# uzh-rpg/dagr

Hardware: NVIDIA H100
Metric: Mevents/sec (higher is better)
Workload: dtype f32

## Files before the change

dagr_b200/_lib.py:

```python
from __future__ import annotations

import ctypes as C
import os
from pathlib import Path

import torch

_PKG = Path(__file__).resolve().parent
_LIB_PATH = Path(os.environ["DAGR_B200_LIB"]) if os.environ.get("DAGR_B200_LIB") else _PKG / "libdagr_b200.so"
_lib = None

ELL = 16
KU = 15
TABW = 16
L1_TC_WFRAG_FLOATS = 8192

p = C.c_void_p
i32 = C.c_int32
i64 = C.c_int64
f32 = C.c_float


class Geom(C.Structure):
    _fields_ = [("W", i32), ("H", i32), ("B", i32), ("T", i32),
                ("r", i32), ("ncell", i32),
                ("dt_us", i32), ("K", i32), ("Q", i32),
                ("nx1", i32), ("ny1", i32),
                ("CW", i32), ("CH", i32), ("CP", i32),
                ("NK", i32),
                ("xkey", p), ("ykey", p), ("spiral", p), ("posx0", p), ("posy0", p), ("vx0", p), ("vy0", p), ("tabx", p), ("taby", p)]


class Grid(C.Structure):
    _fields_ = [("nx", i32), ("ny", i32), ("B", i32), ("W", i32), ("H", i32),
                ("posxr", p), ("posyr", p)]


class EventWs(C.Structure):
    _fields_ = [(k, i64) for k in ("key", "tmp", "count", "blocksums", "start", "perm", "ti", "xyb", "feat_s", "nbr", "off", "cellmask",
                                   "xa", "wl_hdr", "wl_ids", "x1")]


class PoolWs(C.Structure):
    _fields_ = [(k, i64) for k in ("acc", "possum", "ptmax", "pcnt", "pmask")]


class L1AParams(C.Structure):
    _fields_ = [("w", f32 * (KU * 3 * 16)), ("root", f32 * (3 * 16)),
# ... 15 lines not shown
    "dagr_abi_version": (C.c_int, []),
    "dagr_last_error": (C.c_char_p, []),
    "dagr_scan_blocks": (i64, [i64]),
    "dagr_check_config": (C.c_int, [C.POINTER(Geom), i64, C.c_int, C.c_int, C.c_char_p]),
    "dagr_event_workspace_bytes": (C.c_int, [C.POINTER(Geom), i64, C.POINTER(EventWs)]),
    "dagr_pool_workspace_bytes": (C.c_int, [i64, C.c_int, C.POINTER(PoolWs)]),
    "dagr_downsample_events": (C.c_int, [p, p, p, i64, C.c_int, C.c_int, C.c_int, C.c_int, p, p, p, p, p, p, p, p, p]),
    "dagr_compact_events": (C.c_int, [p, i64, p, p, p, p, C.c_int, C.c_int, p, p, p, p, p, p, p, p, p]),
    "dagr_ingest_events": (C.c_int, [p, p, p, p, i64, C.c_int, C.c_int, C.c_int, C.c_int, i64, C.c_int, p, p, p, p, p, p, p, p, p]),
    "dagr_denormalize_pos": (C.c_int, [p, i64, C.c_int, C.c_int, C.c_int, p, p]),
    "dagr_prepare_events": (C.c_int, [p, p, p, C.c_int, i64, C.c_int, C.c_int, C.c_int, p, p, p, p]),
    "dagr_graph_sort": (C.c_int, [C.POINTER(Geom), p, p, p, i64, p, p, p, p, p, p, p, p, p, p, p]),
    "dagr_graph_sort_ring": (C.c_int, [C.POINTER(Geom), p, p, p, i64, p, p, p, p, p, p, p, p, p, p, p, p]),
    "dagr_stream_push": (C.c_int, [p, p, p, p, p, i64, C.c_int, C.c_int, p]),
    "dagr_stream_push_multi": (C.c_int, [p, p, p, p, p, i64, C.c_int, C.c_int, p]),
    "dagr_graph_sort_rings": (C.c_int, [C.POINTER(Geom), p, p, p, i64, C.c_int, p, p, p, p, p, p, p, p, p, p, p, p]),
    "dagr_graph_search": (C.c_int, [C.POINTER(Geom), i64, p, p, p, p, p, p, p]),
    "dagr_l1_build": (C.c_int, [C.POINTER(Geom), i64, p, p, p, p, p, C.POINTER(L1AParams), p, C.c_int, p, p, p, p, p, p, C.c_int, p]),
    "dagr_xa_permute": (C.c_int, [i64, p, C.c_int, p, p, C.c_int, p]),
    "dagr_l1_x0_image": (C.c_int, [C.POINTER(Geom), i64, p, p, p, C.c_int, C.c_int, p, p]),
    "dagr_l1_x0_image_live": (C.c_int, [C.POINTER(Geom), i64, p, p, p, p, C.c_int, C.c_int, p, p]),
    "dagr_l1_conv_a_image": (C.c_int, [C.POINTER(Geom), i64, p, p, p, p, p, p, C.POINTER(L1ImgParams), p, p, p, p, C.c_int, p]),
    "dagr_voxel_sample_max": (C.c_int, [C.POINTER(Geom), i64, p, p, p, C.c_int, C.c_int, C.c_int, p, C.c_int, C.c_int, C.c_int, p]),
    "dagr_graph_export": (C.c_int, [C.POINTER(Geom), i64, p, p, p, p, p, p, p, p, i64, p]),
    "dagr_l1_conv_a": (C.c_int, [C.POINTER(Geom), i64, p, p, p, p, p, C.POINTER(L1AParams), p, p]),
    "dagr_l1_conv_b_pool": (C.c_int, [C.POINTER(Geom), i64, p, p, p, p, p, p, C.POINTER(L1BParams), p, p, p]),
    "dagr_l1_conv_b_pool_voxel": (C.c_int, [C.POINTER(Geom), i64, p, p, p, p, p, p, p, p, C.POINTER(L1BParams), p, C.c_int, p, p, p, p, p, p, p, C.c_int, p, p, C.c_int, p]),
    "dagr_l1_tc_weights": (C.c_int, [p, p, C.c_int, p]),
    "dagr_l1_conv_b_pool_voxel_tc": (C.c_int, [C.POINTER(Geom), i64, p, p, p, p, p, p, p, C.POINTER(L1BParams), p, p, C.c_int, p, p, p, p, p, p, p, C.c_int, p, p, C.c_int, p]),
    "dagr_l1_conv_a_image_tc": (C.c_int, [C.POINTER(Geom), i64, p, p, p, p, p, p, C.POINTER(L1ImgParams), p, p, p, p, p, C.c_int, p]),
    "dagr_pool1_finalize": (C.c_int, [C.POINTER(Geom), i64, p, p, p, p, C.c_int, p, p, p, p, p, p]),
    "dagr_grid_cat_pos": (C.c_int, [C.POINTER(Grid), p, p, p, C.c_int, p, p]),
    "dagr_grid_conv": (C.c_int, [C.POINTER(Grid), p, p, p, p, C.c_int, C.c_int, C.c_int, p, p, p, p, p, p, C.c_int, f32, f32, p, p]),
    "dagr_grid_linear_bn": (C.c_int, [i64, p, p, C.c_int, C.c_int, p, p, p, p, p]),
    "dagr_grid_pool": (C.c_int, [C.POINTER(Grid), C.POINTER(Grid), p, p, p, p, p, p, p, p, C.c_int, C.c_int,
                                 p, p, p, p, p, p, p, p]),
    "dagr_grid_pool_finalize": (C.c_int, [C.POINTER(Grid), C.c_int, C.c_int, p, p, p, p, p, p, p, p, p, p]),
    "dagr_grid_temporal_filter": (C.c_int, [C.POINTER(Grid), p, p, p, p]),
    "dagr_grid_to_dense": (C.c_int, [C.POINTER(Grid), p, p, C.c_int, C.c_int, p, p, p]),
    "dagr_head_decode": (C.c_int, [p, p, p, C.c_int, C.c_int, C.c_int, C.c_int, C.c_int, C.c_int, C.c_int, p, p]),
    "dagr_head_finish": (C.c_int, [C.POINTER(Grid), p, p, C.c_int, p, C.c_int, p, p, p, C.c_int, C.c_int, C.c_int, C.c_int, p, p]),
    "dagr_postprocess_nms": (C.c_int, [p, C.c_int, C.c_int, C.c_int, f32, f32, C.c_int, C.c_int, C.c_int, p, p, p]),
    "dagr_sample_features": (C.c_int, [p, C.c_int, C.c_int, C.c_int, C.c_int, p, p, p, i64, C.c_int, C.c_int, p,
                                       C.c_int, C.c_int, p]),
    "dagr_masked_lin": (C.c_int, [p, i64, p, p, p, p, C.c_int, C.c_int, C.c_int, p]),
    "dagr_masked_inplace_bn": (C.c_int, [p, i64, p, p, p, p, p, p, C.c_int, f32, p]),
    "dagr_masked_isdiff": (C.c_int, [p, i64, p, p, C.c_int, f32, f32, p]),
}

EXPORTS = tuple(_SIGS.keys())


def lib_path() -> Path:
    return _LIB_PATH


def load():
    global _lib
    if _lib is not None:
        return _lib
    if not os.environ.get("DAGR_B200_LIB"):
        from . import build as _build
        if _build.needs_build():
            try:
                _build.build(force=True)
            except Exception as e:
# ... 40 lines not shown
```

dagr_b200/csrc/coarse.cu:

```cuda
#include "common.cuh"

__device__ __forceinline__ float div_floor_f32(float a, float b)
{
    const float mod = fmodf(a, b);
    float div = __fdiv_rn(__fsub_rn(a, mod), b);
    if ((mod != 0.f) && ((b < 0.f) != (mod < 0.f))) div -= 1.f;
    float fl;
    if (div != 0.f) {
        fl = floorf(div);
        if (div - fl > 0.5f) fl += 1.f;
    } else {
        fl = copysignf(0.f, __fdiv_rn(a, b));
    }
    return fl;
}

__device__ __forceinline__ int round_to_pixel(float mean, int size)
{
    const float inv = __frcp_rn((float)size);
    const float q = div_floor_f32(__fadd_rn(mean, 1e-5f), inv);
    const int k = (int)q;
    return min(max(k, 0), size - 1);
}

// ... 284 lines not shown
            const int cell = cell0 + j;
            if (cell >= cells) continue;
            float v = 0.f;
            if (cnt[cell] > 0) {
#pragma unroll
                for (int w2 = 0; w2 < SK_WARPS; w2++) v += part[((size_t)w2 * CPB + j) * Cout + o];
                if (bias) v += bias[o];
                if (scale) v = fmaf(v, scale[o], shift[o]);
                if (skip) v += skip[(int64_t)cell * Cout + o];
                if (relu) v = fmaxf(v, 0.f);
            }
            out[(int64_t)cell * Cout + o] = v;
        }
    }
}

template <int CPB>
static int launch_grid_conv_sk(const dagr_grid_t *gr, const int32_t *cnt, const int32_t *pxy, const uint32_t *mask,
                               const float *xin, int ldin, int Cin, int Cout, const float *weight, const float *rootT, const float *bias,
                               const float *scale, const float *shift, const float *skip, int relu, float den_x, float den_y,
                               float *out, cudaStream_t st)
{
    const int cells = gr->B * gr->ny * gr->nx;
    const size_t a_bytes = (size_t)SK_SLOTS * Cin * CPB * sizeof(float), p_bytes = (size_t)SK_WARPS * CPB * Cout * sizeof(float);
    const size_t smem = (Cout <= 64) ? (a_bytes > p_bytes ? a_bytes : p_bytes) : a_bytes + p_bytes;
    if (smem > 200 * 1024) return -1;
    cudaError_t e = dagr_allow_smem(k_grid_conv_sk<CPB>, smem);
    if (e != cudaSuccess) return -2;
    k_grid_conv_sk<CPB><<<dagr_div_up(cells, CPB), SK_WARPS * 32, smem, st>>>(*gr, cnt, pxy, mask, xin, ldin, Cin, Cout, weight, rootT, bias,
                                                                            scale, shift, skip, relu, den_x, den_y, out);
    return 0;
}

extern "C" int dagr_grid_conv(const dagr_grid_t *gr, const int32_t *cnt, const int32_t *pxy, const uint32_t *mask,
                              const float *xin, int ldin, int Cin, int Cout, const float *weight, const float *rootT,
                              const float *bias, const float *scale, const float *shift, const float *skip, int relu,
                              float den_x, float den_y, float *out, void *stream)
{
    DAGR_CHECK_ARG(gr && Cin > 0 && Cout > 0 && (ldin == 0 || ldin >= Cin), "bad channels");
    if (ldin == 0) ldin = Cin;
    const int cells = gr->B * gr->ny * gr->nx;
    cudaStream_t st = (cudaStream_t)stream;
    static int n_sm = 0;
    if (n_sm == 0) {
        int dev = 0;
        DAGR_CUDA(cudaGetDevice(&dev));
        DAGR_CUDA(cudaDeviceGetAttribute(&n_sm, cudaDevAttrMultiProcessorCount, dev));
    }
    int rc = -1;
    const size_t per_cell = ((size_t)SK_SLOTS * Cin + (Cout <= 64 ? 0 : (size_t)SK_WARPS * Cout)) * sizeof(float);
    if (cells >= n_sm * 16 * 2 && per_cell * 16 <= 110 * 1024)
        rc = launch_grid_conv_sk<16>(gr, cnt, pxy, mask, xin, ldin, Cin, Cout, weight, rootT, bias, scale, shift, skip, relu, den_x, den_y, out, st);
    if (rc != 0 && cells >= n_sm * 4 && per_cell * 4 <= 160 * 1024)
        rc = launch_grid_conv_sk<4>(gr, cnt, pxy, mask, xin, ldin, Cin, Cout, weight, rootT, bias, scale, shift, skip, relu, den_x, den_y, out, st);
    if (rc != 0)
        rc = launch_grid_conv_sk<1>(gr, cnt, pxy, mask, xin, ldin, Cin, Cout, weight, rootT, bias, scale, shift, skip, relu, den_x, den_y, out, st);
    if (rc != 0) {
        const size_t smem = (size_t)GC_WARPS * GC_SLOTS * Cin * sizeof(float);
        DAGR_CHECK_ARG(smem <= 200 * 1024, "Cin too large for the grid conv kernels");
        DAGR_CUDA(dagr_allow_smem(k_grid_conv, smem));
        k_grid_conv<<<dagr_div_up(cells, GC_WARPS), GC_WARPS * 32, smem, st>>>(
            *gr, cnt, pxy, mask, xin, ldin, Cin, Cout, weight, rootT, bias, scale, shift, skip, relu, den_x, den_y, out);
    }
    DAGR_CHECK_LAUNCH();
    return DAGR_OK;
}

#define LB_CELLS 8
__global__ void __launch_bounds__(256)
k_grid_linear_bn(int64_t cells, const int32_t *__restrict__ cnt, const float *__restrict__ xin, int Cin,
                 int Cout, const float *__restrict__ wT, const float *__restrict__ scale,
                 const float *__restrict__ shift, float *__restrict__ out)
{
    extern __shared__ float s_x[];
    __shared__ int s_valid[LB_CELLS];
    const int64_t cell0 = (int64_t)blockIdx.x * LB_CELLS;
    for (int i = threadIdx.x; i < LB_CELLS * Cin; i += blockDim.x) {
        const int64_t cell = cell0 + i / Cin;
        s_x[i] = (cell < cells) ? xin[cell * Cin + i % Cin] : 0.f;
    }
    if (threadIdx.x < LB_CELLS) s_valid[threadIdx.x] = (cell0 + threadIdx.x < cells) && cnt[cell0 + threadIdx.x] > 0;
    __syncthreads();
    const int groups = LB_CELLS / 4;
    for (int t = threadIdx.x; t < Cout * groups; t += blockDim.x) {
        const int o = t % Cout, jg = t / Cout;
        const float *x0 = s_x + (size_t)(4 * jg) * Cin;
        float acc[4] = {0.f, 0.f, 0.f, 0.f};
        for (int c0 = 0; c0 < Cin; c0 += 8) {
            float w[8];
#pragma unroll
            for (int u = 0; u < 8; u++) w[u] = (c0 + u < Cin) ? __ldg(wT + (int64_t)(c0 + u) * Cout + o) : 0.f;
#pragma unroll
            for (int u = 0; u < 8; u++) {
                const int c = min(c0 + u, Cin - 1);
#pragma unroll
                for (int k = 0; k < 4; k++) acc[k] = fmaf(x0[(size_t)k * Cin + c], w[u], acc[k]);
            }
// ... 403 lines not shown
```

dagr_b200/csrc/common.cuh:

```cuda
#pragma once
#include <cuda_runtime.h>
#include <stdint.h>
#include <stdio.h>
#include "../../include/dagr_b200.h"

#ifndef __CUDA_ARCH__
#define DAGR_HOST 1
#endif

void dagr_set_error(const char *fmt, ...);

#define DAGR_CHECK_ARG(cond, msg)                                              \
    do { if (!(cond)) { dagr_set_error("%s: %s", __func__, msg); return DAGR_E_ARG; } } while (0)

#define DAGR_CHECK_LAUNCH()                                                    \
    do { cudaError_t e__ = cudaGetLastError();                                 \
         if (e__ != cudaSuccess) { dagr_set_error("%s: %s", __func__, cudaGetErrorString(e__)); \
                                   return DAGR_E_CUDA; } } while (0)

#define DAGR_CUDA(call)                                                        \
    do { cudaError_t e__ = (call);                                             \
         if (e__ != cudaSuccess) { dagr_set_error("%s: %s", __func__, cudaGetErrorString(e__)); \
                                   return DAGR_E_CUDA; } } while (0)

cudaError_t dagr_allow_smem_impl(const void *kernel, size_t bytes, bool max_carveout);
template <class K> static inline cudaError_t dagr_allow_smem(K kernel, size_t bytes, bool max_carveout = false)
{
    return dagr_allow_smem_impl(reinterpret_cast<const void *>(kernel), bytes, max_carveout);
}

static inline int dagr_div_up(int64_t a, int64_t b) { return (int)((a + b - 1) / b); }

int scan_exclusive(const int *in, int *out, int64_t n, int *blocksums, cudaStream_t st);

#define XA_SWZ(p) ((int)(((p) >> 2) & 1))

__device__ __forceinline__ uint32_t enc_ordered(float f)
{
    uint32_t u = __float_as_uint(f);
    return (u & 0x80000000u) ? ~u : (u | 0x80000000u);
}
__device__ __forceinline__ float dec_ordered(uint32_t e)
{
    uint32_t u = (e & 0x80000000u) ? (e & 0x7fffffffu) : ~e;
    return __uint_as_float(u);
}

__device__ __forceinline__ float2 ffma2(float2 a, float2 b, float2 c) { return make_float2(fmaf(a.x, b.x, c.x), fmaf(a.y, b.y, c.y)); }

__device__ __forceinline__ void spline_basis2(float ax, float ay, int ks, float w[4], int slot[4])
{
    float vx = ax * (float)(ks - 1), vy = ay * (float)(ks - 1);
    float fx = vx - floorf(vx), fy = vy - floorf(vy);
    int ix = (int)vx, iy = (int)vy;
#pragma unroll
    for (int s = 0; s < 4; s++) {
        int kx = s & 1, ky = (s >> 1) & 1;
        int sx = (ix + kx) % ks, sy = (iy + ky) % ks;
        if (sx < 0) sx += ks;
        if (sy < 0) sy += ks;
        slot[s] = sx + ks * sy;
        w[s] = (kx ? fx : 1.f - fx) * (ky ? fy : 1.f - fy);
    }
}
```

dagr_b200/csrc/conv_l1.cu:

```cuda
#include <string.h>
#include "common.cuh"

#define L1_THREADS 128

struct L1Smem {
    float *tab;
    float *posx;
    float *posy;
    short *sp;
};

__device__ __forceinline__ L1Smem l1_smem_init(const dagr_geom_t &g, const float *__restrict__ tab, unsigned char *raw)
{
    L1Smem s;
    s.tab = (float *)raw;
    s.posx = s.tab + g.ncell * DAGR_TABW;
    s.posy = s.posx + g.W;
    s.sp = (short *)(s.posy + g.H);
    for (int i = threadIdx.x; i < g.ncell * DAGR_TABW; i += blockDim.x) s.tab[i] = tab[i];
    for (int i = threadIdx.x; i < g.W; i += blockDim.x) s.posx[i] = g.posx0[i];
    for (int i = threadIdx.x; i < g.H; i += blockDim.x) s.posy[i] = g.posy0[i];
    for (int i = threadIdx.x; i < g.ncell; i += blockDim.x)
        s.sp[i] = (short)(((int)g.spiral[2 * i] & 0xff) | ((int)g.spiral[2 * i + 1] << 8));
    __syncthreads();
// ... 258 lines not shown
    asm volatile("fence.mbarrier_init.release.cluster;" ::: "memory");
}
__device__ __forceinline__ void mbar_expect_tx(uint64_t *bar, uint32_t bytes)
{
    asm volatile("mbarrier.arrive.expect_tx.shared::cta.b64 _, [%0], %1;" ::"r"(smem_u32(bar)), "r"(bytes) : "memory");
}
__device__ __forceinline__ void mbar_wait(uint64_t *bar, uint32_t parity)
{
    asm volatile(
        "{\n"
        ".reg .pred p;\n"
        "WAIT_%=:\n"
        "mbarrier.try_wait.parity.shared::cta.b64 p, [%0], %1;\n"
        "@p bra DONE_%=;\n"
        "bra WAIT_%=;\n"
        "DONE_%=:\n"
        "}\n" ::"r"(smem_u32(bar)), "r"(parity) : "memory");
}
__device__ __forceinline__ void tma_bulk_g2s(void *dst_smem, const void *src_gmem, uint32_t bytes, uint64_t *bar)
{
    asm volatile("cp.async.bulk.shared::cluster.global.mbarrier::complete_tx::bytes [%0], [%1], %2, [%3];" ::"r"(smem_u32(dst_smem)),
                 "l"(src_gmem), "r"(bytes), "r"(smem_u32(bar))
                 : "memory");
}

struct CB2Tile {
    int run_start[3], run_len[3], run_off[3];
};

#ifndef CB2_TC
#define CB2_TC 1
#endif
#define CB2_TC_KSTEPS 16

__device__ __forceinline__ uint32_t tf32_rna(float x)
{
    uint32_t r;
    asm("cvt.rna.tf32.f32 %0, %1;" : "=r"(r) : "f"(x));
    return r;
}
__device__ __forceinline__ void mma_tf32(float2 &c01, float2 &c23, const uint32_t a[4], uint32_t b0, uint32_t b1)
{
    asm("mma.sync.aligned.m16n8k8.row.col.f32.tf32.tf32.f32 {%0, %1, %2, %3}, {%4, %5, %6, %7}, {%8, %9}, {%0, %1, %2, %3};"
        : "+f"(c01.x), "+f"(c01.y), "+f"(c23.x), "+f"(c23.y)
        : "r"(a[0]), "r"(a[1]), "r"(a[2]), "r"(a[3]), "r"(b0), "r"(b1));
}

__device__ __forceinline__ void cb2_tc_kstep(float *xt, const float a[8], const float4 *__restrict__ wf, float2 o2[8])
{
    const int lane = threadIdx.x & 31;
    const float4 w0 = __ldg(wf), w1 = __ldg(wf + 1);
    const uint32_t bh[2][2] = {{__float_as_uint(w0.x), __float_as_uint(w0.y)}, {__float_as_uint(w1.x), __float_as_uint(w1.y)}};
    const uint32_t bl[2][2] = {{__float_as_uint(w0.z), __float_as_uint(w0.w)}, {__float_as_uint(w1.z), __float_as_uint(w1.w)}};
    float *row = xt + 4 * (lane & 15);
    const uint32_t ra = smem_u32(row);
#pragma unroll
    for (int mt = 0; mt < 2; mt++) {
        uint32_t ah[4], al[4];
#pragma unroll
        for (int h = 0; h < 2; h++) {
            __syncwarp();
            if ((lane >> 4) == mt) *reinterpret_cast<float4 *>(row) = make_float4(a[4 * h], a[4 * h + 1], a[4 * h + 2], a[4 * h + 3]);
            __syncwarp();
            uint32_t r0, r1;
            asm volatile("ldmatrix.sync.aligned.m8n8.x2.shared.b16 {%0, %1}, [%2];" : "=r"(r0), "=r"(r1) : "r"(ra) : "memory");
            ah[2 * h] = tf32_rna(__uint_as_float(r0));
            ah[2 * h + 1] = tf32_rna(__uint_as_float(r1));
            al[2 * h] = __float_as_uint(__uint_as_float(r0) - __uint_as_float(ah[2 * h]));
            al[2 * h + 1] = __float_as_uint(__uint_as_float(r1) - __uint_as_float(ah[2 * h + 1]));
        }
        const uint32_t fa[4] = {ah[0], ah[1], ah[2], ah[3]}, fl[4] = {al[0], al[1], al[2], al[3]};
#pragma unroll
        for (int nt = 0; nt < 2; nt++) {
            mma_tf32(o2[4 * mt + 2 * nt], o2[4 * mt + 2 * nt + 1], fl, bh[nt][0], bh[nt][1]);
            mma_tf32(o2[4 * mt + 2 * nt], o2[4 * mt + 2 * nt + 1], fa, bl[nt][0], bl[nt][1]);
            mma_tf32(o2[4 * mt + 2 * nt], o2[4 * mt + 2 * nt + 1], fa, bh[nt][0], bh[nt][1]);
        }
    }
}
// ... 596 lines not shown
                                          persist, x1, cnt, pxy, tmean, tmax, xg, ldx, wl_hdr, wl_ids, defer, (cudaStream_t)stream);
}

template <bool TC>
static int conv_a_image(const dagr_geom_t *g, int64_t N, const int32_t *start, const uint32_t *xyb, const float *feat_s, const float *x0,
                        const int32_t *nbr, const uint16_t *off, const dagr_l1img_params_t *p_host, const float4 *wfrag, float *xa,
                        float *skipv, int32_t *wl_hdr, int32_t *wl_ids, int defer, cudaStream_t st)
{
    DAGR_CHECK_ARG(g && p_host && xyb && feat_s, "null argument");
    if (N <= 0) return DAGR_OK;
    DAGR_CHECK_ARG(g->r <= 15, "radius must be <= 15 px (offsets are packed in 5 bits)");
    return cb2_launch<dagr_l1img_params_t, 2, true, TC>(g, N, start, xyb, nullptr, feat_s, x0, nbr, off, p_host, wfrag, nullptr, 0, nullptr,
                                                        nullptr, nullptr, nullptr, nullptr, nullptr, nullptr, 0, xa, skipv, wl_hdr, wl_ids,
                                                        defer, st);
}

extern "C" int dagr_l1_conv_a_image(const dagr_geom_t *g, int64_t N, const int32_t *start, const uint32_t *xyb, const float *feat_s,
                                    const float *x0, const int32_t *nbr,
                                    const uint16_t *off, const dagr_l1img_params_t *p_host, float *xa, float *skipv,
                                    int32_t *wl_hdr, int32_t *wl_ids, int defer, void *stream)
{
    return conv_a_image<false>(g, N, start, xyb, feat_s, x0, nbr, off, p_host, nullptr, xa, skipv, wl_hdr, wl_ids, defer, (cudaStream_t)stream);
}

extern "C" int dagr_l1_conv_a_image_tc(const dagr_geom_t *g, int64_t N, const int32_t *start, const uint32_t *xyb, const float *feat_s,
                                       const float *x0, const int32_t *nbr, const uint16_t *off, const dagr_l1img_params_t *p_host,
                                       const float *wfrag, float *xa, float *skipv, int32_t *wl_hdr, int32_t *wl_ids, int defer, void *stream)
{
    DAGR_CHECK_ARG(wfrag, "null weight fragments (dagr_l1_tc_weights)");
    return conv_a_image<CB2_TC != 0>(g, N, start, xyb, feat_s, x0, nbr, off, p_host, (const float4 *)wfrag, xa, skipv, wl_hdr, wl_ids, defer,
                                     (cudaStream_t)stream);
}

static float tf32_rna_host(float x)
{
    uint32_t u;
    memcpy(&u, &x, 4);
    if ((u & 0x7f800000u) != 0x7f800000u) u = (u + 0x1000u) & 0xffffe000u;
    float r;
    memcpy(&r, &u, 4);
    return r;
}

extern "C" int dagr_l1_tc_weights(const float *w_host, const float *root_host, int cin, float *wfrag_host)
{
    DAGR_CHECK_ARG(w_host && root_host && wfrag_host, "null argument");
    DAGR_CHECK_ARG(cin >= 16, "the tensor-core instances take input channels 0..15");
    for (int half = 0; half < 2; half++)
        for (int s = 0; s < CB2_TC_KSTEPS; s++)
            for (int lane = 0; lane < 32; lane++)
                for (int nt = 0; nt < 2; nt++) {
                    const int g = lane >> 2, t = lane & 3, n = 8 * nt + g;
                    const float *W = s < DAGR_KU ? w_host + (size_t)s * cin * 16 : root_host;
                    const float x0 = W[(8 * half + t) * 16 + n], x1 = W[(8 * half + t + 4) * 16 + n];
                    const float h0 = tf32_rna_host(x0), h1 = tf32_rna_host(x1);
                    float *o = wfrag_host + ((((size_t)half * CB2_TC_KSTEPS + s) * 32 + lane) * 2 + nt) * 4;
                    o[0] = h0; o[1] = h1; o[2] = x0 - h0; o[3] = x1 - h1;
                }
    return DAGR_OK;
}


__global__ void k_xa_permute(int64_t N, const int32_t *__restrict__ perm, int n_old, float *__restrict__ xa_sorted,
                             float *__restrict__ xa_arrival, int scatter)
{
    const int64_t t = (int64_t)blockIdx.x * blockDim.x + threadIdx.x;
    const int64_t p = t >> 2;
    const int q = (int)(t & 3);
    if (p >= N) return;
    const int i = perm[p];
    float4 *srt = reinterpret_cast<float4 *>(xa_sorted + ((int64_t)(q >> 1) * N + p) * 8) + ((q & 1) ^ XA_SWZ(p));
    float4 *arr = reinterpret_cast<float4 *>(xa_arrival + (int64_t)i * 16) + q;
    if (scatter) { if (i >= n_old) *arr = *srt; }
    else         { if (i < n_old) *srt = *arr; }
}

// ... 8 lines not shown
```

dagr_b200/engine.py:

```python
from __future__ import annotations

import ctypes as C
import math
from typing import Dict, List, Optional

import torch

from . import _lib
from .geometry import Geometry


def _fold_bn(bn):
    m = bn.module
    scale = (m.weight / torch.sqrt(m.running_var + m.eps)).float()
    shift = (m.bias - m.running_mean * scale).float()
    return scale.contiguous(), shift.contiguous()


def _tc_weights(lib, params, cin: int, device) -> torch.Tensor:
    out = (C.c_float * _lib.L1_TC_WFRAG_FLOATS)()
    _lib.check(lib.dagr_l1_tc_weights(C.cast(params.w, C.c_void_p), C.cast(params.root, C.c_void_p), cin, C.cast(out, C.c_void_p)),
               "dagr_l1_tc_weights")
    return torch.frombuffer(out, dtype=torch.float32).clone().to(device)


def _fill(arr, t: torch.Tensor):
    flat = t.detach().float().cpu().contiguous().view(-1)
    assert flat.numel() == len(arr), (flat.numel(), len(arr))
    C.memmove(arr, flat.data_ptr(), flat.numel() * 4)


class _ConvPack:
    def __init__(self, conv, norm=None, relu=False, dev=None):
        self.cin, self.cout = conv.in_channels, conv.out_channels
        self.weight = conv.weight.detach().float().contiguous().to(dev)
        self.rootT = conv.lin.weight.detach().float().t().contiguous().to(dev)
        self.bias = conv.bias.detach().float().contiguous().to(dev) if conv.bias is not None else None
        if norm is not None:
            s, b = _fold_bn(norm)
            self.scale, self.shift = s.detach().to(dev), b.detach().to(dev)
        else:
            self.scale = self.shift = None
        self.relu = relu


def _merge_packs(a: "_ConvPack", b: "_ConvPack") -> "_ConvPack":
    m = _ConvPack.__new__(_ConvPack)
    assert a.cin == b.cin and a.relu == b.relu and (a.bias is None) == (b.bias is None) and (a.scale is None) == (b.scale is None)
    m.cin, m.cout = a.cin, a.cout + b.cout
    m.weight = torch.cat([a.weight, b.weight], dim=2).contiguous()
    m.rootT = torch.cat([a.rootT, b.rootT], dim=1).contiguous()
    m.bias = None if a.bias is None else torch.cat([a.bias, b.bias]).contiguous()
    m.scale = None if a.scale is None else torch.cat([a.scale, b.scale]).contiguous()
    m.shift = None if a.shift is None else torch.cat([a.shift, b.shift]).contiguous()
    m.relu = a.relu
    return m


class _LayerPack:
    def __init__(self, layer, relu, dev):
        self.a = _ConvPack(layer.conv_block1.conv, layer.conv_block1.norm, relu, dev)
        self.b = _ConvPack(layer.conv_block2.conv, layer.conv_block2.norm, relu, dev)
        self.skipT = layer.conv_block2.lin.mlp.weight.detach().float().t().contiguous().to(dev)
        s, b = _fold_bn(layer.conv_block2.norm_skip)
        self.sscale, self.sshift = s.detach().to(dev), b.detach().to(dev)


class GridState:

    def __init__(self, level, cells, dev):
        self.level = level
        self.cells = cells
        self.cnt = torch.empty(cells, dtype=torch.int32, device=dev)
        self.pxy = torch.empty((cells, 2), dtype=torch.int32, device=dev)
        self.tmean = torch.empty(cells, dtype=torch.float32, device=dev)
        self.tmax = torch.empty(cells, dtype=torch.float32, device=dev)
        self.mask = None
        self.x = None


class _WsView:
    _SLOT_KEYS = ("zero_buf", "grids", "pool", "graph", "graph_warm", "graph_key")

    def __init__(self, base: dict, slot: dict):
# ... 9 lines not shown
        return k in (self.slot if k in self._SLOT_KEYS else self.base)

    def get(self, k, default=None):
        return (self.slot if k in self._SLOT_KEYS else self.base).get(k, default)


class Engine:
    def __init__(self, model):
        self.model = model
        self.lib = _lib.load()
        self._geoms: Dict[tuple, Geometry] = {}
        self._pack = None
        self._pack_key = None
        self._pack_gen = 0
        self._sentinels = None
        self._ws: Dict[tuple, dict] = {}
        self.keep_node_features = False
        self.voxel_conv_b = True
        self.use_graphs = True
        self.fused_build = True
        self.dense_worklists = "auto"
        self._dense = {}
        self.last = {}
        self.launches = 0
        self.prof = None
        self.overlap = False
        self._cstream = None
        self._fstream = None
        self._slot = 0
        self._done = [None, None]
        self._out_slot = {}

    _NKERNELS = dict(dagr_graph_sort=6, dagr_graph_sort_ring=6, dagr_stream_push=2, dagr_graph_sort_rings=6, dagr_stream_push_multi=2, dagr_graph_search=1, dagr_l1_build=2, dagr_graph_export=5, dagr_l1_conv_a=1, dagr_l1_conv_b_pool=1, dagr_l1_conv_b_pool_voxel=2, dagr_l1_conv_b_pool_voxel_tc=2, dagr_l1_x0_image=1, dagr_l1_x0_image_live=1, dagr_xa_permute=1, dagr_l1_conv_a_image=2, dagr_l1_conv_a_image_tc=2, dagr_voxel_sample_max=1,
                     dagr_pool1_finalize=1, dagr_grid_cat_pos=1, dagr_grid_conv=1, dagr_grid_linear_bn=1, dagr_grid_pool=1,
                     dagr_grid_pool_finalize=1, dagr_grid_temporal_filter=1, dagr_grid_to_dense=1, dagr_head_decode=1, dagr_head_finish=1,
                     dagr_postprocess_nms=1, dagr_sample_features=1, dagr_denormalize_pos=1)

    def _run(self, label, fn, *args):
        if self.prof is not None:
            e0 = torch.cuda.Event(enable_timing=True); e1 = torch.cuda.Event(enable_timing=True)
            e0.record()
        _lib.check(fn(*args), label)
        self.launches += self._NKERNELS.get(fn.__name__, 1)
        if self.prof is not None:
            e1.record()
            self.prof.setdefault(label, []).append((e0, e1))

    def prof_summary(self):
        out = {}
        for k, evs in (self.prof or {}).items():
            ts = [a.elapsed_time(b) for a, b in evs]
            out[k] = dict(ms=sum(ts) / len(ts), calls=len(ts))
        return out

    def geometry(self, W, H, B, device) -> Geometry:
        key = (int(W), int(H), int(B), str(device))
        g = self._geoms.get(key)
        if g is None:
            a = self.model.args
            g = Geometry(W, H, B, radius=a.radius, time_window=self.model.time_window,
                         max_neighbors=a.max_neighbors, max_queue_size=self.model.backbone.events_to_graph.max_queue_size,
                         pooling_dim_at_output=a.pooling_dim_at_output, kernel_size=getattr(a, "kernel_size", 5),
                         device=device)
            self._geoms[key] = g
        return g

    def _params_key(self):
# ... 192 lines not shown
                    st["defer"][k], st["quiet"][k] = 1, 0
                elif st["defer"][k]:
                    st["quiet"][k] += 1
                    if st["quiet"][k] >= 16:
                        st["defer"][k] = 0
            st["event"] = None
        return list(st["defer"])

    def _dense_report(self, ws, wl_hdr):
        st = self._dense.get(id(ws.base))
        if st is None or st["event"] is not None:
            return
        st["host"].copy_(wl_hdr[:8], non_blocking=True)
        ev = torch.cuda.Event()
        ev.record()
        st["event"] = ev

    def _zs(self, ws, name, dtype):
        off, nbytes = ws["zero_slices"][name]
        return ws["zero_buf"][off:off + nbytes].view(dtype)

    def _buf(self, ws, name, shape, dtype, dev):
        t = ws["pool"].get(name)
        n = 1
        for s in shape:
            n *= s
        if t is None or t.numel() < n or t.dtype != dtype:
            t = torch.empty(max(n, 1), dtype=dtype, device=dev)
            ws["pool"][name] = t
        return t[:n].view(*shape)

    def _grid_conv(self, geom, lv, gs: GridState, xin, pack: _ConvPack, skip, out, st, ldin=0):
        level = geom.levels[lv]
        self._run(f"grid_conv_L{lv + 1}_{pack.cin}x{pack.cout}", self.lib.dagr_grid_conv, C.byref(level.grid), _lib.ptr(gs.cnt), _lib.ptr(gs.pxy), _lib.ptr(gs.mask),
                                           _lib.ptr(xin), int(ldin), pack.cin, pack.cout, _lib.ptr(pack.weight), _lib.ptr(pack.rootT),
                                           _lib.ptr(pack.bias), _lib.ptr(pack.scale), _lib.ptr(pack.shift),
                                           _lib.ptr(skip), 1 if pack.relu else 0, level.den_x, level.den_y,
                                           _lib.ptr(out), st)

    def _layer(self, geom, lv, gs: GridState, lp: _LayerPack, ws, name, st, dev):
        level = geom.levels[lv]
        cells = gs.cells
        cx = gs.x.shape[1]
        xin = self._buf(ws, name + "_in", (cells, cx + 2), torch.float32, dev)
        self._run("cat_pos", self.lib.dagr_grid_cat_pos, C.byref(level.grid), _lib.ptr(gs.cnt), _lib.ptr(gs.pxy), _lib.ptr(gs.x), cx,
                                              _lib.ptr(xin), st)
        a = self._buf(ws, name + "_a", (cells, lp.a.cout), torch.float32, dev)
        self._grid_conv(geom, lv, gs, xin, lp.a, None, a, st)
        sk = self._buf(ws, name + "_s", (cells, lp.b.cout), torch.float32, dev)
        self._run("linear_bn", self.lib.dagr_grid_linear_bn, cells, _lib.ptr(gs.cnt), _lib.ptr(xin), cx + 2, lp.b.cout,
                                                _lib.ptr(lp.skipT), _lib.ptr(lp.sscale), _lib.ptr(lp.sshift),
                                                _lib.ptr(sk), st)
        out = self._buf(ws, name + "_o", (cells, lp.b.cout), torch.float32, dev)
        self._grid_conv(geom, lv, gs, a, lp.b, sk, out, st)
        return xin, a, out

    def _pool(self, geom, lv_child, gc: GridState, x, aggr, ws, st, dev, keep_temporal):
        lp = lv_child + 1
        child, parent = geom.levels[lv_child], geom.levels[lp]
        gp: GridState = ws["grids"][lp]
        Cc = x.shape[1]
        acc = self._zs(ws, f"acc{lp}", torch.uint8)
        if gp.cells * Cc * 8 > acc.numel():
            raise RuntimeError(f"dagr_b200: pooling accumulator of level {lp + 1} holds {acc.numel()} bytes, {gp.cells * Cc * 8} needed "
                               f"({Cc} channels)")
        accmax = acc.view(torch.int32) if aggr == 0 else None
        accsum = acc.view(torch.float64) if aggr == 1 else None
        possum = self._zs(ws, f"possum{lp}", torch.float64)
# ... 325 lines not shown
```

include/dagr_b200.h:

```cpp
#ifndef DAGR_B200_H
#define DAGR_B200_H

#include <stdint.h>
#include <stddef.h>

#ifdef __cplusplus
extern "C" {
#endif

#define DAGR_ABI_VERSION 2

#define DAGR_OK            0
#define DAGR_E_ARG        -1
#define DAGR_E_CUDA       -2
#define DAGR_E_UNSUPPORTED -3

#define DAGR_ELL 16
#define DAGR_KU  15
#define DAGR_TABW 16
#define DAGR_RING_CTL 8

int         dagr_abi_version(void);
const char *dagr_last_error(void);

// ... 145 lines not shown
int dagr_l1_tc_weights(const float *w_host ,
                       const float *root_host , int cin ,
                       float *wfrag_host );
int dagr_l1_conv_b_pool_voxel_tc(const dagr_geom_t *g, int64_t N, const int32_t *start, const uint32_t *xyb,
                                 const int32_t *ti, const float *feat_s, const float *xa, const int32_t *nbr,
                                 const uint16_t *off, const dagr_l1b_params_t *p_host, const float *wfrag,
                                 const float *skip_pre, int min_idx, float *persist,
                                 float *x1, int32_t *cnt, int32_t *pxy, float *tmean, float *tmax, float *xg, int ldx,
                                 int32_t *wl_hdr, int32_t *wl_ids, int defer, void *stream);
int dagr_l1_conv_a_image_tc(const dagr_geom_t *g, int64_t N, const int32_t *start, const uint32_t *xyb, const float *feat_s,
                            const float *x0, const int32_t *nbr, const uint16_t *off, const dagr_l1img_params_t *p_host,
                            const float *wfrag, float *xa, float *skipv, int32_t *wl_hdr, int32_t *wl_ids, int defer, void *stream);

typedef struct {
    int32_t nx, ny, B;
    int32_t W, H;
    const float *posxr;
    const float *posyr;
} dagr_grid_t;

int dagr_pool1_finalize(const dagr_geom_t *g, int64_t N, const int32_t *start, const uint32_t *xyb,
                        const int32_t *ti, const uint32_t *poolmax, int C,
                        int32_t *cnt, int32_t *pxy, float *tmean, float *tmax, float *x, void *stream);

int dagr_grid_cat_pos(const dagr_grid_t *gr, const int32_t *cnt, const int32_t *pxy, const float *x,
                      int Cx, float *xin, void *stream);

int dagr_grid_conv(const dagr_grid_t *gr, const int32_t *cnt, const int32_t *pxy, const uint32_t *mask,
                   const float *xin, int ldin ,
                   int Cin, int Cout, const float *weight, const float *rootT,
                   const float *bias, const float *scale, const float *shift, const float *skip,
                   int relu, float den_x, float den_y, float *out, void *stream);

int dagr_grid_linear_bn(int64_t cells, const int32_t *cnt, const float *xin, int Cin, int Cout,
                        const float *wT, const float *scale, const float *shift,
                        float *out, void *stream);

int dagr_grid_pool(const dagr_grid_t *child, const dagr_grid_t *parent, const int32_t *cellx,
                   const int32_t *celly, const int32_t *cnt, const int32_t *pxy, const float *tmean,
                   const float *tmax, const uint32_t *mask, const float *x, int C, int aggr,
                   uint32_t *accmax, double *accsum, double *possum, uint32_t *ptmax, int32_t *pcnt,
                   uint32_t *pmask, int32_t *err_flag, void *stream);

int dagr_grid_pool_finalize(const dagr_grid_t *parent, int C, int aggr, const uint32_t *accmax,
                            const double *accsum, const double *possum, const uint32_t *ptmax,
                            const int32_t *pcnt, int32_t *pxy, float *tmean, float *tmax, float *x,
                            void *stream);

int dagr_grid_temporal_filter(const dagr_grid_t *gr, const int32_t *cnt, const float *tmax,
                              uint32_t *mask, void *stream);

int dagr_grid_to_dense(const dagr_grid_t *gr, const int32_t *cnt, const float *x, int C, int ldx ,
                       const float *add , float *dense, void *stream);

int dagr_head_decode(const float *reg, const float *obj, const float *cls, int B, int nc, int h, int w,
                     int stride, int a0, int A, float *out, void *stream);

int dagr_head_finish(const dagr_grid_t *gr, const int32_t *cnt, const float *cls, int ldc, const float *regobj, int ldr,
                     const float *add_cls, const float *add_reg, const float *add_obj, int nc, int stride, int a0, int A,
                     float *out, void *stream);

int dagr_postprocess_nms(const float *pred, int B, int A, int nc, float conf_thre, float nms_thre,
                         int width, int height, int filtering, float *det, int32_t *ndet, void *stream);

int dagr_sample_features(const float *img, int Bi, int C, int h, int w, const float *posx, const float *posy,
                         const int32_t *bidx, int64_t n, int width, int height, float *out, int ldo, int c0,
// ... 26 lines not shown
```

Baseline: 545.7.

## Add 3xTF32 tensor-core spline conv kernel for coarse grid layers

Adds a tensor-core grid convolution that builds, per spline slot, a gathered and weighted neighbour feature tile in shared memory (double-buffered). It multiplies that tile by pre-fragmented weights with split-TF32 mma (three MMAs per step) to keep roughly fp32 accuracy. Weight fragments are precomputed on the host once per layer. It is used only for large grids with Cin >= 32, and falls back to the fp32 kernel otherwise. The goal is to replace scalar FMA work in the coarse convs with tensor-core throughput, at the cost of extra gather work, per-slot block syncs and a tripled MMA count.

```diff
diff --git a/dagr_b200/_lib.py b/dagr_b200/_lib.py
--- a/dagr_b200/_lib.py
+++ b/dagr_b200/_lib.py
@@ -14,6 +14,11 @@
 KU = 15
 TABW = 16
 L1_TC_WFRAG_FLOATS = 8192
+
+
+def grid_tc_wfrag_floats(cin: int, cout: int) -> int:
+    return 52 * ((cin + 7) // 8 * 8) * ((cout + 7) // 8 * 8)
+
 
 p = C.c_void_p
 i32 = C.c_int32
@@ -95,6 +100,8 @@
     "dagr_pool1_finalize": (C.c_int, [C.POINTER(Geom), i64, p, p, p, p, C.c_int, p, p, p, p, p, p]),
     "dagr_grid_cat_pos": (C.c_int, [C.POINTER(Grid), p, p, p, C.c_int, p, p]),
     "dagr_grid_conv": (C.c_int, [C.POINTER(Grid), p, p, p, p, C.c_int, C.c_int, C.c_int, p, p, p, p, p, p, C.c_int, f32, f32, p, p]),
+    "dagr_grid_tc_weights": (C.c_int, [p, p, C.c_int, C.c_int, p]),
+    "dagr_grid_conv_tc": (C.c_int, [C.POINTER(Grid), p, p, p, p, C.c_int, C.c_int, C.c_int, p, p, p, p, p, p, p, C.c_int, f32, f32, p, p]),
     "dagr_grid_linear_bn": (C.c_int, [i64, p, p, C.c_int, C.c_int, p, p, p, p, p]),
     "dagr_grid_pool": (C.c_int, [C.POINTER(Grid), C.POINTER(Grid), p, p, p, p, p, p, p, p, C.c_int, C.c_int,
                                  p, p, p, p, p, p, p, p]),
diff --git a/dagr_b200/csrc/coarse.cu b/dagr_b200/csrc/coarse.cu
--- a/dagr_b200/csrc/coarse.cu
+++ b/dagr_b200/csrc/coarse.cu
@@ -340,21 +340,25 @@
     return 0;
 }
 
-extern "C" int dagr_grid_conv(const dagr_grid_t *gr, const int32_t *cnt, const int32_t *pxy, const uint32_t *mask,
-                              const float *xin, int ldin, int Cin, int Cout, const float *weight, const float *rootT,
-                              const float *bias, const float *scale, const float *shift, const float *skip, int relu,
-                              float den_x, float den_y, float *out, void *stream)
-{
-    DAGR_CHECK_ARG(gr && Cin > 0 && Cout > 0 && (ldin == 0 || ldin >= Cin), "bad channels");
-    if (ldin == 0) ldin = Cin;
-    const int cells = gr->B * gr->ny * gr->nx;
-    cudaStream_t st = (cudaStream_t)stream;
+static int grid_sm_count()
+{
     static int n_sm = 0;
     if (n_sm == 0) {
         int dev = 0;
-        DAGR_CUDA(cudaGetDevice(&dev));
-        DAGR_CUDA(cudaDeviceGetAttribute(&n_sm, cudaDevAttrMultiProcessorCount, dev));
-    }
+        if (cudaGetDevice(&dev) != cudaSuccess || cudaDeviceGetAttribute(&n_sm, cudaDevAttrMultiProcessorCount, dev) != cudaSuccess)
+            return 0;
+    }
+    return n_sm;
+}
+
+static int grid_conv_fp32(const dagr_grid_t *gr, const int32_t *cnt, const int32_t *pxy, const uint32_t *mask,
+                          const float *xin, int ldin, int Cin, int Cout, const float *weight, const float *rootT,
+                          const float *bias, const float *scale, const float *shift, const float *skip, int relu,
+                          float den_x, float den_y, float *out, cudaStream_t st)
+{
+    const int cells = gr->B * gr->ny * gr->nx;
+    const int n_sm = grid_sm_count();
+    DAGR_CHECK_ARG(n_sm > 0, "no CUDA device");
     int rc = -1;
     const size_t per_cell = ((size_t)SK_SLOTS * Cin + (Cout <= 64 ? 0 : (size_t)SK_WARPS * Cout)) * sizeof(float);
     if (cells >= n_sm * 16 * 2 && per_cell * 16 <= 110 * 1024)
@@ -371,6 +375,214 @@
             *gr, cnt, pxy, mask, xin, ldin, Cin, Cout, weight, rootT, bias, scale, shift, skip, relu, den_x, den_y, out);
     }
     DAGR_CHECK_LAUNCH();
+    return DAGR_OK;
+}
+
+extern "C" int dagr_grid_conv(const dagr_grid_t *gr, const int32_t *cnt, const int32_t *pxy, const uint32_t *mask,
+                              const float *xin, int ldin, int Cin, int Cout, const float *weight, const float *rootT,
+                              const float *bias, const float *scale, const float *shift, const float *skip, int relu,
+                              float den_x, float den_y, float *out, void *stream)
+{
+    DAGR_CHECK_ARG(gr && Cin > 0 && Cout > 0 && (ldin == 0 || ldin >= Cin), "bad channels");
+    return grid_conv_fp32(gr, cnt, pxy, mask, xin, ldin ? ldin : Cin, Cin, Cout, weight, rootT, bias, scale, shift, skip, relu,
+                          den_x, den_y, out, (cudaStream_t)stream);
+}
+
+#define GT_WARPS 8
+
+template <int MT>
+__global__ void __launch_bounds__(GT_WARPS * 32, 2)
+k_grid_conv_tc(const dagr_grid_t gr, const int32_t *__restrict__ cnt, const int32_t *__restrict__ pxy,
+               const uint32_t *__restrict__ mask, const float *__restrict__ xin, int ldin, int Cin, int Cout,
+               const float4 *__restrict__ wfrag, const float *__restrict__ bias, const float *__restrict__ scale,
+               const float *__restrict__ shift, const float *__restrict__ skip, int relu, float den_x, float den_y,
+               float *__restrict__ out)
+{
+    constexpr int M = 16 * MT;
+    extern __shared__ __align__(16) float smem_f[];
+    __shared__ int s_src[8][M];
+    __shared__ float s_w[8][4][M];
+    __shared__ uint32_t s_km[GC_SLOTS][M];
+    __shared__ unsigned int s_used;
+    const int Kpad = (Cin + 7) & ~7, lda = Kpad + 4;
+    const int KS = Kpad >> 3, NT = (Cout + 7) >> 3;
+    const int cells = gr.B * gr.ny * gr.nx;
+    const int cell0 = blockIdx.x * M;
+    const int tid = threadIdx.x, lane = tid & 31, warp = tid >> 5;
+    const int per = gr.ny * gr.nx;
+
+    if (tid == 0) s_used = 1u << GC_SLOTS;
+    for (int i = tid; i < GC_SLOTS * M; i += blockDim.x) (&s_km[0][0])[i] = 0u;
+    __syncthreads();
+    for (int i = tid; i < M * 8; i += blockDim.x) {
+        const int j = i >> 3, e = i & 7, bit = e < 4 ? e : e + 1;
+        const int cell = cell0 + j;
+        int src = -1;
+        if (cell < cells && cnt[cell] > 0 && ((mask[cell] >> bit) & 1u)) {
+            const int b = cell / per, rem = cell % per, cy = rem / gr.nx, cx = rem % gr.nx;
+            const int sx = cx + bit % 3 - 1, sy = cy + bit / 3 - 1;
+            if (sx >= 0 && sy >= 0 && sx < gr.nx && sy < gr.ny && cnt[b * per + sy * gr.nx + sx] > 0) src = b * per + sy * gr.nx + sx;
+        }
+        s_src[e][j] = src;
+        if (src >= 0) {
+            const int dx = pxy[2 * src] - pxy[2 * cell], dy = pxy[2 * src + 1] - pxy[2 * cell + 1];
+            const float ax = __fadd_rn(__fdiv_rn((float)dx, den_x), 0.5f);
+            const float ay = __fadd_rn(__fdiv_rn((float)dy, den_y), 0.5f);
+            float w[4]; int slot[4];
+            spline_basis2(ax, ay, 5, w, slot);
+            unsigned int used = 0;
+#pragma unroll
+            for (int q = 0; q < 4; q++) {
+                s_w[e][q][j] = w[q];
+                if (w[q] != 0.f) {
+                    atomicOr(&s_km[slot[q]][j], (1u << e) | ((unsigned int)q << (8 + 2 * e)));
+                    used |= 1u << slot[q];
+                }
+            }
+            atomicOr(&s_used, used);
+        }
+    }
+    __syncthreads();
+
+    const int mt = warp % MT, nt0 = blockIdx.y * 8 + (warp / MT) * MT;
+    const int g = lane >> 2, t = lane & 3;
+    const bool active = nt0 < NT;
+    float2 run[MT][2];
+#pragma unroll
+    for (int i = 0; i < MT; i++) run[i][0] = run[i][1] = make_float2(0.f, 0.f);
+    int buf = 0;
+    for (unsigned int u = s_used; u; u &= u - 1, buf ^= 1) {
+        const int k = __ffs(u) - 1;
+        float *A = smem_f + (size_t)buf * M * lda;
+        for (int j = warp; j < M; j += GT_WARPS) {
+            const int cell = cell0 + j;
+            const uint32_t word = k < GC_SLOTS ? s_km[k][j] : 0u;
+            const bool root = k == GC_SLOTS && cell < cells && cnt[cell] > 0;
+            for (int c = lane; c < Kpad; c += 32) {
+                float a = 0.f;
+                if (c < Cin) {
+                    if (root) a = xin[(int64_t)cell * ldin + c];
+                    for (uint32_t m = word & 0xffu; m; m &= m - 1) {
+                        const int e = __ffs(m) - 1, q = (word >> (8 + 2 * e)) & 3u;
+                        a = fmaf(s_w[e][q][j], xin[(int64_t)s_src[e][j] * ldin + c], a);
+                    }
+                }
+                A[j * lda + c] = a;
+            }
+        }
+        __syncthreads();
+        if (active) {
+            float2 fr[MT][2];
+#pragma unroll
+            for (int i = 0; i < MT; i++) fr[i][0] = fr[i][1] = make_float2(0.f, 0.f);
+            const float *Ar = A + (16 * mt + g) * lda + t;
+            const float4 *wk = wfrag + (size_t)k * KS * NT * 32 + lane;
+            for (int ks = 0; ks < KS; ks++) {
+                const float av[4] = {Ar[8 * ks], Ar[8 * lda + 8 * ks], Ar[8 * ks + 4], Ar[8 * lda + 8 * ks + 4]};
+                uint32_t ah[4], al[4];
+#pragma unroll
+                for (int r = 0; r < 4; r++) {
+                    ah[r] = tf32_rna(av[r]);
+                    al[r] = __float_as_uint(av[r] - __uint_as_float(ah[r]));
+                }
+#pragma unroll
+                for (int i = 0; i < MT; i++) {
+                    if (nt0 + i >= NT) continue;
+                    const float4 w = __ldg(wk + ((size_t)ks * NT + nt0 + i) * 32);
+                    const uint32_t bh0 = __float_as_uint(w.x), bh1 = __float_as_uint(w.y);
+                    const uint32_t bl0 = __float_as_uint(w.z), bl1 = __float_as_uint(w.w);
+                    mma_tf32(fr[i][0], fr[i][1], al, bh0, bh1);
+                    mma_tf32(fr[i][0], fr[i][1], ah, bl0, bl1);
+                    mma_tf32(fr[i][0], fr[i][1], ah, bh0, bh1);
+                }
+            }
+#pragma unroll
+            for (int i = 0; i < MT; i++)
+#pragma unroll
+                for (int h = 0; h < 2; h++)
+                    run[i][h] = make_float2(__fadd_rn(run[i][h].x, fr[i][h].x), __fadd_rn(run[i][h].y, fr[i][h].y));
+        }
+    }
+    if (!active) return;
+#pragma unroll
+    for (int i = 0; i < MT; i++) {
+        if (nt0 + i >= NT) continue;
+#pragma unroll
+        for (int h = 0; h < 2; h++) {
+            const int cell = cell0 + 16 * mt + g + 8 * h;
+            if (cell >= cells) continue;
+            const bool valid = cnt[cell] > 0;
+#pragma unroll
+            for (int p = 0; p < 2; p++) {
+                const int o = 8 * (nt0 + i) + 2 * t + p;
+                if (o >= Cout) continue;
+                float v = 0.f;
+                if (valid) {
+                    v = p ? run[i][h].y : run[i][h].x;
+                    if (bias) v += bias[o];
+                    if (scale) v = fmaf(v, scale[o], shift[o]);
+                    if (skip) v += skip[(int64_t)cell * Cout + o];
+                    if (relu) v = fmaxf(v, 0.f);
+                }
+                out[(int64_t)cell * Cout + o] = v;
+            }
+        }
+    }
+}
+
+template <int MT>
+static int launch_grid_conv_tc(const dagr_grid_t *gr, const int32_t *cnt, const int32_t *pxy, const uint32_t *mask,
+                               const float *xin, int ldin, int Cin, int Cout, const float4 *wfrag, const float *bias,
+                               const float *scale, const float *shift, const float *skip, int relu, float den_x, float den_y,
+                               float *out, cudaStream_t st)
+{
+    const int cells = gr->B * gr->ny * gr->nx;
+    const size_t smem = (size_t)2 * 16 * MT * (((Cin + 7) & ~7) + 4) * sizeof(float);
+    if (smem > 160 * 1024) return -1;
+    if (dagr_allow_smem(k_grid_conv_tc<MT>, smem) != cudaSuccess) return -2;
+    const dim3 grid(dagr_div_up(cells, 16 * MT), dagr_div_up(Cout, 64));
+    k_grid_conv_tc<MT><<<grid, GT_WARPS * 32, smem, st>>>(*gr, cnt, pxy, mask, xin, ldin, Cin, Cout, wfrag, bias, scale, shift, skip,
+                                                           relu, den_x, den_y, out);
+    return 0;
+}
+
+extern "C" int dagr_grid_conv_tc(const dagr_grid_t *gr, const int32_t *cnt, const int32_t *pxy, const uint32_t *mask,
+                                 const float *xin, int ldin, int Cin, int Cout, const float *weight, const float *rootT,
+                                 const float *wfrag, const float *bias, const float *scale, const float *shift, const float *skip,
+                                 int relu, float den_x, float den_y, float *out, void *stream)
+{
+    DAGR_CHECK_ARG(gr && Cin > 0 && Cout > 0 && (ldin == 0 || ldin >= Cin), "bad channels");
+    DAGR_CHECK_ARG(wfrag, "null weight fragments (dagr_grid_tc_weights)");
+    if (ldin == 0) ldin = Cin;
+    cudaStream_t st = (cudaStream_t)stream;
+    const float4 *wf = (const float4 *)wfrag;
+    int rc = -1;
+    if (gr->ny * gr->nx >= 2048 && Cin >= 32)
+        rc = launch_grid_conv_tc<1>(gr, cnt, pxy, mask, xin, ldin, Cin, Cout, wf, bias, scale, shift, skip, relu, den_x, den_y, out, st);
+    if (rc != 0)
+        return grid_conv_fp32(gr, cnt, pxy, mask, xin, ldin, Cin, Cout, weight, rootT, bias, scale, shift, skip, relu, den_x, den_y, out, st);
+    DAGR_CHECK_LAUNCH();
+    return DAGR_OK;
+}
+
+extern "C" int dagr_grid_tc_weights(const float *weight, const float *rootT, int Cin, int Cout, float *wfrag)
+{
+    DAGR_CHECK_ARG(weight && rootT && wfrag, "null argument");
+    DAGR_CHECK_ARG(Cin > 0 && Cout > 0, "bad channels");
+    const int KS = (Cin + 7) / 8, NT = (Cout + 7) / 8;
+    for (int k = 0; k < SK_SLOTS; k++) {
+        const float *W = k < GC_SLOTS ? weight + (size_t)k * Cin * Cout : rootT;
+        for (int ks = 0; ks < KS; ks++)
+            for (int nt = 0; nt < NT; nt++)
+                for (int lane = 0; lane < 32; lane++) {
+                    const int n = 8 * nt + (lane >> 2), c0 = 8 * ks + (lane & 3), c1 = c0 + 4;
+                    const float x0 = (c0 < Cin && n < Cout) ? W[(size_t)c0 * Cout + n] : 0.f;
+                    const float x1 = (c1 < Cin && n < Cout) ? W[(size_t)c1 * Cout + n] : 0.f;
+                    const float h0 = tf32_rna_host(x0), h1 = tf32_rna_host(x1);
+                    float *o = wfrag + ((((size_t)k * KS + ks) * NT + nt) * 32 + lane) * 4;
+                    o[0] = h0; o[1] = h1; o[2] = x0 - h0; o[3] = x1 - h1;
+                }
+    }
     return DAGR_OK;
 }
 
diff --git a/dagr_b200/csrc/common.cuh b/dagr_b200/csrc/common.cuh
--- a/dagr_b200/csrc/common.cuh
+++ b/dagr_b200/csrc/common.cuh
@@ -2,6 +2,7 @@
 #include <cuda_runtime.h>
 #include <stdint.h>
 #include <stdio.h>
+#include <string.h>
 #include "../../include/dagr_b200.h"
 
 #ifndef __CUDA_ARCH__
@@ -48,6 +49,28 @@
 
 __device__ __forceinline__ float2 ffma2(float2 a, float2 b, float2 c) { return make_float2(fmaf(a.x, b.x, c.x), fmaf(a.y, b.y, c.y)); }
 
+__device__ __forceinline__ uint32_t tf32_rna(float x)
+{
+    uint32_t r;
+    asm("cvt.rna.tf32.f32 %0, %1;" : "=r"(r) : "f"(x));
+    return r;
+}
+__device__ __forceinline__ void mma_tf32(float2 &c01, float2 &c23, const uint32_t a[4], uint32_t b0, uint32_t b1)
+{
+    asm("mma.sync.aligned.m16n8k8.row.col.f32.tf32.tf32.f32 {%0, %1, %2, %3}, {%4, %5, %6, %7}, {%8, %9}, {%0, %1, %2, %3};"
+        : "+f"(c01.x), "+f"(c01.y), "+f"(c23.x), "+f"(c23.y)
+        : "r"(a[0]), "r"(a[1]), "r"(a[2]), "r"(a[3]), "r"(b0), "r"(b1));
+}
+static inline float tf32_rna_host(float x)
+{
+    uint32_t u;
+    memcpy(&u, &x, 4);
+    if ((u & 0x7f800000u) != 0x7f800000u) u = (u + 0x1000u) & 0xffffe000u;
+    float r;
+    memcpy(&r, &u, 4);
+    return r;
+}
+
 __device__ __forceinline__ void spline_basis2(float ax, float ay, int ks, float w[4], int slot[4])
 {
     float vx = ax * (float)(ks - 1), vy = ay * (float)(ks - 1);
diff --git a/dagr_b200/csrc/conv_l1.cu b/dagr_b200/csrc/conv_l1.cu
--- a/dagr_b200/csrc/conv_l1.cu
+++ b/dagr_b200/csrc/conv_l1.cu
@@ -314,19 +314,6 @@
 #define CB2_TC 1
 #endif
 #define CB2_TC_KSTEPS 16
-
-__device__ __forceinline__ uint32_t tf32_rna(float x)
-{
-    uint32_t r;
-    asm("cvt.rna.tf32.f32 %0, %1;" : "=r"(r) : "f"(x));
-    return r;
-}
-__device__ __forceinline__ void mma_tf32(float2 &c01, float2 &c23, const uint32_t a[4], uint32_t b0, uint32_t b1)
-{
-    asm("mma.sync.aligned.m16n8k8.row.col.f32.tf32.tf32.f32 {%0, %1, %2, %3}, {%4, %5, %6, %7}, {%8, %9}, {%0, %1, %2, %3};"
-        : "+f"(c01.x), "+f"(c01.y), "+f"(c23.x), "+f"(c23.y)
-        : "r"(a[0]), "r"(a[1]), "r"(a[2]), "r"(a[3]), "r"(b0), "r"(b1));
-}
 
 __device__ __forceinline__ void cb2_tc_kstep(float *xt, const float a[8], const float4 *__restrict__ wf, float2 o2[8])
 {
@@ -989,16 +976,6 @@
                                      (cudaStream_t)stream);
 }
 
-static float tf32_rna_host(float x)
-{
-    uint32_t u;
-    memcpy(&u, &x, 4);
-    if ((u & 0x7f800000u) != 0x7f800000u) u = (u + 0x1000u) & 0xffffe000u;
-    float r;
-    memcpy(&r, &u, 4);
-    return r;
-}
-
 extern "C" int dagr_l1_tc_weights(const float *w_host, const float *root_host, int cin, float *wfrag_host)
 {
     DAGR_CHECK_ARG(w_host && root_host && wfrag_host, "null argument");
diff --git a/dagr_b200/engine.py b/dagr_b200/engine.py
--- a/dagr_b200/engine.py
+++ b/dagr_b200/engine.py
@@ -30,11 +30,19 @@
     C.memmove(arr, flat.data_ptr(), flat.numel() * 4)
 
 
+def _grid_tc_weights(weight: torch.Tensor, rootT: torch.Tensor, cin: int, cout: int) -> torch.Tensor:
+    w, r = weight.detach().float().cpu().contiguous(), rootT.detach().float().cpu().contiguous()
+    out = torch.empty(_lib.grid_tc_wfrag_floats(cin, cout), dtype=torch.float32)
+    _lib.check(_lib.load().dagr_grid_tc_weights(_lib.ptr(w), _lib.ptr(r), cin, cout, _lib.ptr(out)), "dagr_grid_tc_weights")
+    return out.to(weight.device)
+
+
 class _ConvPack:
     def __init__(self, conv, norm=None, relu=False, dev=None):
         self.cin, self.cout = conv.in_channels, conv.out_channels
         self.weight = conv.weight.detach().float().contiguous().to(dev)
         self.rootT = conv.lin.weight.detach().float().t().contiguous().to(dev)
+        self.wfrag = _grid_tc_weights(self.weight, self.rootT, self.cin, self.cout)
         self.bias = conv.bias.detach().float().contiguous().to(dev) if conv.bias is not None else None
         if norm is not None:
             s, b = _fold_bn(norm)
@@ -50,6 +58,7 @@
     m.cin, m.cout = a.cin, a.cout + b.cout
     m.weight = torch.cat([a.weight, b.weight], dim=2).contiguous()
     m.rootT = torch.cat([a.rootT, b.rootT], dim=1).contiguous()
+    m.wfrag = _grid_tc_weights(m.weight, m.rootT, m.cin, m.cout)
     m.bias = None if a.bias is None else torch.cat([a.bias, b.bias]).contiguous()
     m.scale = None if a.scale is None else torch.cat([a.scale, b.scale]).contiguous()
     m.shift = None if a.shift is None else torch.cat([a.shift, b.shift]).contiguous()
@@ -125,7 +134,7 @@
         self._out_slot = {}
 
     _NKERNELS = dict(dagr_graph_sort=6, dagr_graph_sort_ring=6, dagr_stream_push=2, dagr_graph_sort_rings=6, dagr_stream_push_multi=2, dagr_graph_search=1, dagr_l1_build=2, dagr_graph_export=5, dagr_l1_conv_a=1, dagr_l1_conv_b_pool=1, dagr_l1_conv_b_pool_voxel=2, dagr_l1_conv_b_pool_voxel_tc=2, dagr_l1_x0_image=1, dagr_l1_x0_image_live=1, dagr_xa_permute=1, dagr_l1_conv_a_image=2, dagr_l1_conv_a_image_tc=2, dagr_voxel_sample_max=1,
-                     dagr_pool1_finalize=1, dagr_grid_cat_pos=1, dagr_grid_conv=1, dagr_grid_linear_bn=1, dagr_grid_pool=1,
+                     dagr_pool1_finalize=1, dagr_grid_cat_pos=1, dagr_grid_conv=1, dagr_grid_conv_tc=1, dagr_grid_linear_bn=1, dagr_grid_pool=1,
                      dagr_grid_pool_finalize=1, dagr_grid_temporal_filter=1, dagr_grid_to_dense=1, dagr_head_decode=1, dagr_head_finish=1,
                      dagr_postprocess_nms=1, dagr_sample_features=1, dagr_denormalize_pos=1)
 
@@ -384,8 +393,9 @@
 
     def _grid_conv(self, geom, lv, gs: GridState, xin, pack: _ConvPack, skip, out, st, ldin=0):
         level = geom.levels[lv]
-        self._run(f"grid_conv_L{lv + 1}_{pack.cin}x{pack.cout}", self.lib.dagr_grid_conv, C.byref(level.grid), _lib.ptr(gs.cnt), _lib.ptr(gs.pxy), _lib.ptr(gs.mask),
+        self._run(f"grid_conv_L{lv + 1}_{pack.cin}x{pack.cout}", self.lib.dagr_grid_conv_tc, C.byref(level.grid), _lib.ptr(gs.cnt), _lib.ptr(gs.pxy), _lib.ptr(gs.mask),
                                            _lib.ptr(xin), int(ldin), pack.cin, pack.cout, _lib.ptr(pack.weight), _lib.ptr(pack.rootT),
+                                           _lib.ptr(pack.wfrag),
                                            _lib.ptr(pack.bias), _lib.ptr(pack.scale), _lib.ptr(pack.shift),
                                            _lib.ptr(skip), 1 if pack.relu else 0, level.den_x, level.den_y,
                                            _lib.ptr(out), st)
diff --git a/include/dagr_b200.h b/include/dagr_b200.h
--- a/include/dagr_b200.h
+++ b/include/dagr_b200.h
@@ -201,6 +201,14 @@
                    const float *bias, const float *scale, const float *shift, const float *skip,
                    int relu, float den_x, float den_y, float *out, void *stream);
 
+#define DAGR_GRID_TC_WFRAG_FLOATS(cin, cout) (52 * (((cin) + 7) / 8 * 8) * (((cout) + 7) / 8 * 8))
+int dagr_grid_tc_weights(const float *weight , const float *rootT , int Cin, int Cout,
+                         float *wfrag_host );
+int dagr_grid_conv_tc(const dagr_grid_t *gr, const int32_t *cnt, const int32_t *pxy, const uint32_t *mask,
+                      const float *xin, int ldin, int Cin, int Cout, const float *weight, const float *rootT,
+                      const float *wfrag, const float *bias, const float *scale, const float *shift, const float *skip,
+                      int relu, float den_x, float den_y, float *out, void *stream);
+
 int dagr_grid_linear_bn(int64_t cells, const int32_t *cnt, const float *xin, int Cin, int Cout,
                         const float *wT, const float *scale, const float *shift,
                         float *out, void *stream);
```

New measurement: 559.0, median of 6. 1.02x the previous value.
